# Plonky3/Plonky3

Measured on NVIDIA B200. Metric: coset_lde_batch output Gelem/s (KoalaBear 2^20 x 100 per GPU, blowup 2), higher is better.
Workload: dtype u32 (31-bit Montgomery)

## Files before the change

plonky3_b200/csrc/ntt.cu:

```cuda
#include <algorithm>
#include <cstdio>
#include <cstdlib>
#include <cstring>
#include <vector>

#include <cuda.h>

#include "common.h"

namespace p3 {

#ifdef P3GPU_NTT_PROFILE
#define P3_SKIP(flag) (flag)
#else
#define P3_SKIP(flag) false
#endif

static int env_int(const char *name, int dflt) {
    const char *s = getenv(name);
    return s ? atoi(s) : dflt;
}

struct PassArgs {
    const u32 *in;
// ... 214 lines not shown
            cp_async8(tws + k, tw + ((size_t)1 << (a.l0 + lam)) + ((size_t)T << lam) + ql);
        }
    };
    auto issue = [&](u32 t, u32 buf) {
        u32 coset, col, cw, T, ibase;
        decode(t, coset, col, cw, T, ibase);
        u32 *data = data0 + buf * buf_words;
        const u32 *in = a.in + (size_t)coset * a.in_stride + col;
        if (!shared_tw || a.n_cosets > 1) issue_twiddles(coset, T, tws0 + buf * R);
        const u32 cpr = vec16 ? (cw >> 2) : cw;
        const u32 rs = (THREADS / cpr) & ~(E2 - 1u);
        const u32 nthr = rs * cpr;
        if (rs == 0) {
            for (u32 it = threadIdx.x; it < R * cpr; it += THREADS) {
                const u32 rho = it / cpr, ch = it - rho * cpr;
                const u32 e = vec16 ? 4u * ch : ch;
                const u32 i = ibase | (rho << lowbits);
                const u32 row = a.in_bitrev ? (__brev(i) >> brsh) : i;
                u32 *dst = data + (rho >> Q2) * gstride + (rho & (E2 - 1u)) * CT + e;
                const u32 *src = in + (size_t)row * a.w + e;
                if (vec16) cp_async16(dst, src); else cp_async4(dst, src);
            }
        } else if (threadIdx.x < nthr) {
            const u32 rho0 = threadIdx.x / cpr, ch = threadIdx.x - rho0 * cpr;
            const u32 e = vec16 ? 4u * ch : ch;
            u32 *dst = data + (rho0 >> Q2) * gstride + (rho0 & (E2 - 1u)) * CT + e;
            const u32 dstep = (rs >> Q2) * gstride;
            if (!a.in_bitrev) {
                const u32 *src = in + (size_t)(ibase | (rho0 << lowbits)) * a.w + e;
                const size_t sstep = ((size_t)rs << lowbits) * a.w;
                for (u32 rho = rho0; rho < R; rho += rs, dst += dstep, src += sstep) {
                    if (vec16) cp_async16(dst, src); else cp_async4(dst, src);
                }
            } else {
                for (u32 rho = rho0; rho < R; rho += rs, dst += dstep) {
                    const u32 row = __brev(ibase | (rho << lowbits)) >> brsh;
                    const u32 *src = in + (size_t)row * a.w + e;
                    if (vec16) cp_async16(dst, src); else cp_async4(dst, src);
                }
            }
        }
        cp_async_commit();
    };

    u32 t = blockIdx.x;
    if (t >= total) return;
#ifdef P3GPU_NTT_PROFILE
#define P3_STAMP(slot) do { if (a.prof && threadIdx.x == 0 && k < 16) { unsigned long long ts_; asm volatile("mov.u64 %0, %%globaltimer;" : "=l"(ts_)); \
        a.prof[((size_t)blockIdx.x * 16 + k) * 8 + (slot)] = ts_; } } while (0)
#else
#define P3_STAMP(slot) do { } while (0)
#endif
    if (shared_tw && a.n_cosets == 1) issue_twiddles(0, 0, tws0);
    if (NBUF == 2) issue(t, 0);
    for (u32 k = 0; t < total; t += gridDim.x, k++) {
        const u32 buf = NBUF == 2 ? (k & 1u) : 0u;
        __syncthreads();
#ifdef P3GPU_NTT_PROFILE
        if (a.prof && threadIdx.x == 0 && k < 16) { u32 sm_; asm volatile("mov.u32 %0, %%smid;" : "=r"(sm_)); a.prof[((size_t)blockIdx.x * 16 + k) * 8] = sm_; }
#endif
        P3_STAMP(1);
        if (NBUF == 2) {
            if (t + gridDim.x < total) { issue(t + gridDim.x, buf ^ 1u); cp_async_wait<1>(); }
            else cp_async_wait<0>();
        } else {
            if (!P3_SKIP(a.skip_load)) issue(t, 0);
            P3_STAMP(2);
            cp_async_wait<0>();
        }
        __syncthreads();
        P3_STAMP(3);
        u32 *data = data0 + buf * buf_words;
        const uint2 *tws = (shared_tw && a.n_cosets == 1) ? tws0 : tws0 + buf * R;
        u32 coset, col, cw, T, ibase;
        decode(t, coset, col, cw, T, ibase);
        const u32 dg = THREADS / cw, dc = THREADS - dg * cw;
        {
            u32 g = threadIdx.x / cw, c = threadIdx.x - g * cw;
            for (; g < E2; ) {
                u32 *sp = data + g * CT + c;
                u32 x[E1];
#pragma unroll
                for (u32 m = 0; m < E1; m++) x[m] = sp[m * gstride];
                if (a.has_scale) {
#pragma unroll
                    for (u32 m = 0; m < E1; m++) x[m] = shoup_mul<F>(x[m], a.scale);
                }
                if (!P3_SKIP(a.skip_bfly)) reg_network<F, Q1>(x, tws, 1u);
#pragma unroll
                for (u32 m = 0; m < E1; m++) sp[m * gstride] = x[m];
                c += dc; g += dg;
                if (c >= cw) { c -= cw; g++; }
            }
        }
        __syncthreads();
        P3_STAMP(4);
        {
            u32 *out = a.out + (size_t)coset * a.out_stride + col;
            const size_t sstride = ((size_t)(a.out_bitrev ? (1u << (a.l0 + Q1)) : (1u << lowbits)) << a.out_sh) * a.w;
            u32 g = threadIdx.x / cw, c = threadIdx.x - g * cw;
            for (; g < E1; ) {
                u32 *sp = data + g * gstride + c;
                u32 x[E2];
#pragma unroll
                for (u32 m = 0; m < E2; m++) x[m] = sp[m * CT];
                if (!P3_SKIP(a.skip_bfly)) reg_network<F, Q2>(x, tws, E1 + g);
                if (a.final_reduce) {
#pragma unroll
                    for (u32 m = 0; m < E2; m++) x[m] = fp_reduce<F>(x[m]);
                }
                {
                    const u32 i0 = ibase | (g << (lowbits + Q2));
                    const u32 row0 = ((a.out_bitrev ? (__brev(i0) >> brsh) : i0) << a.out_sh) + a.out_add;
                    u32 *p = out + (size_t)row0 * a.w + c;
                    if (P3_SKIP(a.skip_store)) { u32 acc = 0;
#pragma unroll
                        for (u32 m = 0; m < E2; m++) acc ^= x[m];
                        if (acc == 0x12345678u) p[0] = acc;
                    } else if (a.out_bitrev) {
#pragma unroll
                        for (u32 m = 0; m < E2; m++) p[brev_const<Q2>(m) * sstride] = x[m];
                    } else {
#pragma unroll
                        for (u32 m = 0; m < E2; m++) p[m * sstride] = x[m];
                    }
                }
                c += dc; g += dg;
                if (c >= cw) { c -= cw; g++; }
            }
        }
        P3_STAMP(5);
    }
}

__device__ __forceinline__ void mbar_init(u32 bar, u32 count) { asm volatile("mbarrier.init.shared::cta.b64 [%0], %1;" ::"r"(bar), "r"(count)); }
__device__ __forceinline__ void mbar_wait(u32 bar, u32 parity) {
    u32 done = 0, spins = 0;
    unsigned long long t0 = 0;
    while (true) {
        asm volatile("{ .reg .pred p; mbarrier.try_wait.parity.shared::cta.b64 p, [%1], %2; selp.u32 %0, 1, 0, p; }" : "=r"(done) : "r"(bar), "r"(parity) : "memory");
        if (done) break;
        if ((++spins & 0xfffu) == 0) {
            unsigned long long now;
            asm volatile("mov.u64 %0, %%globaltimer;" : "=l"(now));
            if (t0 == 0) t0 = now;
            else if (now - t0 > 20000000000ull) __trap();
        }
    }
}
__device__ __forceinline__ void mbar_arrive(u32 bar) { asm volatile("mbarrier.arrive.shared::cta.b64 _, [%0];" ::"r"(bar) : "memory"); }
__device__ __forceinline__ void mbar_arrive_n(u32 bar, u32 n) { asm volatile("mbarrier.arrive.shared::cta.b64 _, [%0], %1;" ::"r"(bar), "r"(n) : "memory"); }
__device__ __forceinline__ void mbar_expect_tx(u32 bar, u32 bytes) { asm volatile("mbarrier.arrive.expect_tx.shared::cta.b64 _, [%0], %1;" ::"r"(bar), "r"(bytes) : "memory"); }

template <int F, int R_LOG, bool PERM, int NSTAGE, int NGROUP, int GTHREADS>
__global__ void __launch_bounds__(NGROUP * GTHREADS + 32, 1) ntt_pass_pipe_kernel(const __grid_constant__ CUtensorMap tmap, const __grid_constant__ PassArgs a) {
    constexpr u32 CT = 8;
    constexpr int Q2 = (R_LOG + 1) / 2, Q1 = R_LOG - Q2;
    constexpr u32 E1 = 1u << Q1, E2 = 1u << Q2, R = 1u << R_LOG;
    constexpr u32 GS = PERM ? E1 : E2, NG = PERM ? E2 : E1;
    constexpr u32 gstride = (GS + 1) * CT;
    constexpr u32 STAGE_WORDS = NG * gstride;
    constexpr u32 BOX_BYTES = STAGE_WORDS * 4;
    static_assert(BOX_BYTES % 128 == 0, "stage alignment");
    extern __shared__ __align__(128) unsigned char smem_raw[];
    u32 *stages = reinterpret_cast<u32 *>(smem_raw);
    uint2 *tws0 = reinterpret_cast<uint2 *>(smem_raw + (size_t)NSTAGE * BOX_BYTES);
    const u32 bar0 = (u32)__cvta_generic_to_shared(smem_raw + (size_t)NSTAGE * BOX_BYTES + 2 * R * sizeof(uint2));
    auto full_bar = [&](u32 s) { return bar0 + 8u * s; };
    auto empty_bar = [&](u32 s) { return bar0 + 8u * (NSTAGE + s); };
    auto twfull_bar = [&](u32 b) { return bar0 + 8u * (2 * NSTAGE + b); };
    auto twempty_bar = [&](u32 b) { return bar0 + 8u * (2 * NSTAGE + 2 + b); };

    if (threadIdx.x == 0) {
        for (u32 s = 0; s < NSTAGE; s++) { mbar_init(full_bar(s), 1); mbar_init(empty_bar(s), NGROUP * GTHREADS); }
        for (u32 b = 0; b < 2; b++) { mbar_init(twfull_bar(b), 1); mbar_init(twempty_bar(b), a.tpi * NGROUP * GTHREADS); }
        asm volatile("fence.mbarrier_init.release.cluster;" ::: "memory");
    }
    __syncthreads();

    const int lowbits = a.log_n - a.l1;
    const int brsh = 32 - a.log_n;
    auto decode = [&](u32 it, u32 &coset, u32 &L, u32 &T, u32 &ct0, u32 &ct1) {
        const u32 unit = it / a.csplit, chunk = it - unit * a.csplit;
        coset = unit % a.n_cosets;
        const u32 tile = unit / a.n_cosets;
        L = tile & ((1u << lowbits) - 1u);
        T = tile >> lowbits;
        ct0 = chunk * a.tpi;
        ct1 = min(ct0 + a.tpi, a.n_ctiles);
    };

    if (threadIdx.x >= NGROUP * GTHREADS) {
        if ((threadIdx.x & 31u) != 0) return;
        u32 q = 0, ui = 0;
        for (u32 it = blockIdx.x; it < a.n_items; it += gridDim.x, ui++) {
            u32 coset, L, T, ct0, ct1;
            decode(it, coset, L, T, ct0, ct1);
            const u32 b = ui & 1u, ph = (ui >> 1) & 1u;
            mbar_wait(twempty_bar(b), ph ^ 1u);
            if (ct1 - ct0 < a.tpi) mbar_arrive_n(twempty_bar(b), (a.tpi - (ct1 - ct0)) * NGROUP * GTHREADS);
            {
                const uint2 *tw = a.tw + (size_t)coset * a.tw_stride;
                uint2 *tws = tws0 + b * R;
                tws[1] = tw[((size_t)1 << a.l0) + T];
                mbar_expect_tx(twfull_bar(b), 8u * (R - 2u));
#pragma unroll 1
                for (int lam = 1; lam < R_LOG; lam++) {
                    const uint2 *src = tw + ((size_t)1 << (a.l0 + lam)) + ((size_t)T << lam);
                    asm volatile("cp.async.bulk.shared::cluster.global.mbarrier::complete_tx::bytes [%0], [%1], %2, [%3];"
                                 ::"r"((u32)__cvta_generic_to_shared(tws + (1u << lam))), "l"(src), "r"(8u << lam), "r"(twfull_bar(b)) : "memory");
                }
            }
            const u32 in_block = (a.in_tiled ? a.in_blocks > 1 : a.in_stride != 0) ? coset : 0u;
            const int blk_sh = PERM ? lowbits : a.l0;
            const int c3 = PERM ? 0 : (int)L;
            const int c4 = (PERM ? (lowbits ? (int)(__brev(L) >> (32 - lowbits)) : 0) : (int)T) + (int)(in_block << blk_sh);
            for (u32 ct = ct0; ct < ct1; ct++, q++) {
                const u32 s = q % NSTAGE, k = q / NSTAGE;
                mbar_wait(empty_bar(s), (k & 1u) ^ 1u);
                mbar_expect_tx(full_bar(s), BOX_BYTES);
                const int cc0 = a.in_tiled ? 0 : (int)(ct * CT);
                const int cc4 = a.in_tiled ? c4 + (int)((ct * a.in_blocks) << blk_sh) : c4;
                asm volatile("cp.async.bulk.tensor.5d.shared::cluster.global.mbarrier::complete_tx::bytes [%0], [%1, {%2, %3, %4, %5, %6}], [%7];"
                             ::"r"((u32)__cvta_generic_to_shared(stages + (size_t)s * STAGE_WORDS)), "l"(reinterpret_cast<unsigned long long>(&tmap)),
                               "r"(cc0), "r"(0), "r"(0), "r"(c3), "r"(cc4), "r"(full_bar(s)) : "memory");
            }
        }
        return;
    }

    const u32 gid = threadIdx.x / GTHREADS, tg = threadIdx.x - gid * GTHREADS;
    u32 q = 0, ui = 0;
#ifdef P3GPU_NTT_PROFILE
    u32 kk = 0;
#define P3_GSTAMP(slot) do { if (a.prof && tg == 0 && kk < 16) { unsigned long long ts_; asm volatile("mov.u64 %0, %%globaltimer;" : "=l"(ts_)); \
        a.prof[(((size_t)blockIdx.x * NGROUP + gid) * 16 + kk) * 8 + (slot)] = ts_; } } while (0)
#else
#define P3_GSTAMP(slot) do { } while (0)
#endif
    for (u32 it = blockIdx.x; it < a.n_items; it += gridDim.x, ui++) {
        u32 coset, L, T, ct0, ct1;
        decode(it, coset, L, T, ct0, ct1);
        const u32 b = ui & 1u, ph = (ui >> 1) & 1u;
        const uint2 *tws = tws0 + b * R;
        const u32 ibase = (a.l0 == 0 ? 0u : (T << (a.log_n - a.l0))) | L;
        bool tw_ready = false;
        for (u32 ct = ct0; ct < ct1; ct++, q++) {
            const u32 s = q % NSTAGE, k = q / NSTAGE;
            const u32 col = ct * CT, cw = min(CT, a.wc - col);
            u32 *data = stages + (size_t)s * STAGE_WORDS;
            P3_GSTAMP(1);
            mbar_wait(full_bar(s), k & 1u);
            if (!tw_ready) { mbar_wait(twfull_bar(b), ph); tw_ready = true; }
            if (q % NGROUP != gid) {
                mbar_arrive(empty_bar(s));
                mbar_arrive(twempty_bar(b));
                continue;
            }
            P3_GSTAMP(2);
            const u32 dg = GTHREADS / cw, dc = GTHREADS - dg * cw;
            {
                u32 g = tg / cw, c = tg - g * cw;
                for (; g < E2; ) {
                    u32 x[E1];
                    if (!PERM) {
                        u32 *sp = data + g * CT + c;
#pragma unroll
                        for (u32 m = 0; m < E1; m++) x[m] = sp[m * gstride];
                        if (a.has_scale) {
#pragma unroll
                            for (u32 m = 0; m < E1; m++) x[m] = shoup_mul<F>(x[m], a.scale);
                        }
                        reg_network<F, Q1>(x, tws, 1u);
#pragma unroll
                        for (u32 m = 0; m < E1; m++) sp[m * gstride] = x[m];
                    } else {
                        u32 *sp = data + g * gstride + c;
#pragma unroll
                        for (u32 m = 0; m < E1; m++) x[m] = sp[brev_const<Q1>(m) * CT];
                        if (a.has_scale) {
#pragma unroll
                            for (u32 m = 0; m < E1; m++) x[m] = shoup_mul<F>(x[m], a.scale);
                        }
                        reg_network<F, Q1>(x, tws, 1u);
#pragma unroll
                        for (u32 m = 0; m < E1; m++) sp[brev_const<Q1>(m) * CT] = x[m];
                    }
                    c += dc; g += dg;
                    if (c >= cw) { c -= cw; g++; }
                }
            }
            asm volatile("bar.sync %0, %1;" ::"r"(gid + 1u), "r"((u32)GTHREADS) : "memory");
            P3_GSTAMP(3);
            {
                const u32 ow = a.out_tiled ? CT : a.w;
                u32 *out = a.out_tiled ? a.out + ((((size_t)ct * a.n_cosets + coset) << a.log_n) << 3) : a.out + (size_t)coset * a.out_stride + col;
                const size_t sstride = ((size_t)(a.out_bitrev ? (1u << (a.l0 + Q1)) : (1u << lowbits)) << a.out_sh) * ow;
                u32 g = tg / cw, c = tg - g * cw;
                bool released = false;
                for (; g < E1; ) {
                    u32 x[E2];
                    u32 gg;
                    if (!PERM) {
                        gg = g;
                        const u32 *sp = data + g * gstride + c;
#pragma unroll
                        for (u32 m = 0; m < E2; m++) x[m] = sp[m * CT];
                    } else {
                        gg = __brev(g) >> (32 - Q1);
                        const u32 *sp = data + g * CT + c;
#pragma unroll
                        for (u32 m = 0; m < E2; m++) x[m] = sp[brev_const<Q2>(m) * gstride];
                    }
                    u32 gn = g + dg, cn = c + dc;
                    if (cn >= cw) { cn -= cw; gn++; }
                    if (gn >= E1) {
                        asm volatile("fence.proxy.async.shared::cta;" ::: "memory");
                        mbar_arrive(empty_bar(s));
                        released = true;
                    }
                    reg_network<F, Q2>(x, tws, E1 + gg);
                    if (a.final_reduce) {
#pragma unroll
                        for (u32 m = 0; m < E2; m++) x[m] = fp_reduce<F>(x[m]);
                    }
                    const u32 i0 = ibase | (gg << (lowbits + Q2));
                    const u32 row0 = ((a.out_bitrev ? (__brev(i0) >> brsh) : i0) << a.out_sh) + a.out_add;
                    u32 *p = out + (size_t)row0 * ow + c;
                    if (a.shard_log_rows) {
                        const u32 grow = (coset << a.log_n) + row0;
                        p = a.shard_out[grow >> a.shard_log_rows] + (size_t)(grow & ((1u << a.shard_log_rows) - 1u)) * ow + col + c;
                    }
                    if (a.out_bitrev) {
#pragma unroll
                        for (u32 m = 0; m < E2; m++) p[brev_const<Q2>(m) * sstride] = x[m];
                    } else {
#pragma unroll
                        for (u32 m = 0; m < E2; m++) p[m * sstride] = x[m];
                    }
                    g = gn; c = cn;
                }
                if (!released) {
                    asm volatile("fence.proxy.async.shared::cta;" ::: "memory");
                    mbar_arrive(empty_bar(s));
                }
            }
            mbar_arrive(twempty_bar(b));
            P3_GSTAMP(4);
#ifdef P3GPU_NTT_PROFILE
            kk++;
#endif
        }
    }
}

struct TwGenArgs {
    u32 sigma[32];
    u32 roots[32];
};
template <int F> __global__ void gen_twiddle_heap(uint2 *Z, int log_n, const TwGenArgs a) {
    const size_t idx = (size_t)blockIdx.x * blockDim.x + threadIdx.x;
    if (idx >= ((size_t)1 << log_n)) return;
    if (idx == 0) { Z[0] = make_uint2(0, 0); return; }
    const int l = 63 - __clzll((long long)idx);
    const u32 q = (u32)(idx - ((size_t)1 << l));
    u32 z = a.sigma[l];
    for (int b = 0; b < l; b++)
        if ((q >> b) & 1u) z = mont_mul<F>(z, a.roots[b + 2]);
    Z[idx] = shoup_pair<F>(from_monty<F>(z));
}

struct PowArgs { u32 pw[32]; };
template <int F> __global__ void scale_rows_by_powers(u32 *m, size_t h, size_t w, const PowArgs a) {
    const size_t idx = (size_t)blockIdx.x * blockDim.x + threadIdx.x;
    if (idx >= h * w) return;
    size_t row = idx / w;
    u32 s = Fp<F>::ONE;
    for (int k = 0; row; k++, row >>= 1)
        if (row & 1) s = mont_mul<F>(s, a.pw[k]);
    m[idx] = mont_mul<F>(m[idx], s);
}
__global__ void broadcast_row(const u32 *in, u32 *out, size_t rows, size_t w) {
    const size_t idx = (size_t)blockIdx.x * blockDim.x + threadIdx.x;
    if (idx < rows * w) out[idx] = in[idx % w];
}

template <int F>
static int32_t get_twiddles(p3gpu_ctx *ctx, int log_n, int added_bits, u32 shift, int inverse, const uint2 **out) {
    TwiddleKey key{F, log_n, shift, inverse + 2 * added_bits};
    std::lock_guard<std::recursive_mutex> g(ctx->call_mu);
    {
        auto it = ctx->twiddles.find(key);
        if (it != ctx->twiddles.end()) { it->second.last_use = ctx->tick; *out = it->second.ptr; return P3GPU_OK; }
    }
    const size_t N = (size_t)1 << log_n, n_cosets = (size_t)1 << added_bits;
    const size_t bytes = n_cosets * N * sizeof(uint2);
    while (ctx->twiddle_bytes + bytes > ctx->twiddle_cap_bytes) {
        auto victim = ctx->twiddles.end();
        for (auto it = ctx->twiddles.begin(); it != ctx->twiddles.end(); ++it)
            if (it->second.last_use < ctx->tick && (victim == ctx->twiddles.end() || it->second.last_use < victim->second.last_use)) victim = it;
        if (victim == ctx->twiddles.end()) break;
        P3_CUDA(cudaStreamSynchronize(ctx->stream));
        P3_CUDA(cudaFree(victim->second.ptr));
        ctx->twiddle_bytes -= victim->second.bytes;
        ctx->twiddles.erase(victim);
    }
    uint2 *Z = nullptr;
    {
        cudaError_t e = cudaMalloc(&Z, bytes);
        if (e != cudaSuccess) { set_error("cudaMalloc(%zu) for a twiddle heap failed: %s", bytes, cudaGetErrorString(e)); cudaGetLastError(); return P3GPU_ENOMEM; }
    }
    const u32 g_big = two_adic_generator<F>((u32)(log_n + added_bits));
    for (size_t cb = 0; cb < n_cosets; cb++) {
        size_t c = 0;
        for (int b = 0; b < added_bits; b++) c |= ((cb >> b) & 1) << (added_bits - 1 - b);
        const u32 s = mont_mul<F>(shift, fp_pow<F>(g_big, c));
        TwGenArgs a;
        for (int l = 0; l < 32; l++) { a.sigma[l] = Fp<F>::ONE; a.roots[l] = Fp<F>::ONE; }
        for (int l = 0; l < log_n; l++) a.sigma[l] = fp_pow<F>(s, (u64)(N >> (l + 1)));
        for (u32 k = 0; k <= (u32)log_n && k <= Fp<F>::TWO_ADICITY; k++) {
            u32 gk = two_adic_generator<F>(k);
            a.roots[k] = inverse ? fp_inv<F>(gk) : gk;
        }
        const unsigned blocks = (unsigned)((N + 255) / 256);
        gen_twiddle_heap<F><<<blocks, 256, 0, ctx->stream>>>(Z + cb * N, log_n, a);
        ctx->launches++;
        const cudaError_t e = cudaGetLastError();
        if (e != cudaSuccess) { cudaFree(Z); set_error("gen_twiddle_heap launch failed: %s", cudaGetErrorString(e)); return P3GPU_ECUDA; }
    }
    ctx->twiddles.emplace(key, TwiddleEntry{Z, bytes, ctx->tick});
    ctx->twiddle_bytes += bytes;
    *out = Z;
    return P3GPU_OK;
}

template <int F, int LOG_CT, bool VEC>
static int32_t launch_pass_ct(p3gpu_ctx *ctx, const PassArgs &a) {
    constexpr int THREADS = 256;
    const int r = a.l1 - a.l0;
    const size_t smem = (((size_t)1 << r) << LOG_CT) * 4 + ((size_t)1 << r) * sizeof(uint2);
    auto kern = ntt_pass_kernel<F, LOG_CT, THREADS, VEC>;
    if (smem > 48 * 1024) P3_CUDA(cudaFuncSetAttribute(kern, cudaFuncAttributeMaxDynamicSharedMemorySize, (int)smem));
    const size_t tiles = ((size_t)1 << (a.log_n - r)) * a.n_ctiles * a.n_cosets;
    P3_CHECK(tiles < (1ull << 31), P3GPU_EINVAL, "ntt: grid too large");
    kern<<<(unsigned)tiles, THREADS, smem, ctx->stream>>>(a);
    ctx->launches++;
    P3_CUDA(cudaGetLastError());
    return P3GPU_OK;
}

template <int F, int R_LOG, int CT_T, int THREADS, int NBUF>
static int32_t launch_fast_rct(p3gpu_ctx *ctx, const PassArgs &a) {
    constexpr int Q2 = (R_LOG + 1) / 2, Q1 = R_LOG - Q2;
    const u32 ct = a.ct;
    const u32 e2 = 1u << Q2, e1 = 1u << Q1;
    const u32 padw = (ct + 32u - ((e2 * ct) & 31u)) & 31u;
    const size_t buf_words = ((size_t)e1 * (e2 * ct + padw) + 3) & ~(size_t)3;
    const size_t smem = NBUF * buf_words * 4 + NBUF * ((size_t)1 << R_LOG) * sizeof(uint2);
    auto kern = ntt_pass_fast_kernel<F, R_LOG, CT_T, THREADS, NBUF>;
    P3_CHECK(smem <= 227 * 1024, P3GPU_EINVAL, "ntt: tile does not fit shared memory");
    static size_t smem_set[64] = {0};
    if (smem > 48 * 1024 && smem > smem_set[ctx->device & 63]) {
        P3_CUDA(cudaFuncSetAttribute(kern, cudaFuncAttributeMaxDynamicSharedMemorySize, (int)smem));
        smem_set[ctx->device & 63] = smem;
    }
    const size_t tiles = ((size_t)1 << (a.log_n - R_LOG)) * a.n_ctiles * a.n_cosets;
    P3_CHECK(tiles < (1ull << 31), P3GPU_EINVAL, "ntt: grid too large");
    size_t per_sm = std::min<size_t>(NBUF == 1 ? 2048 / THREADS : 2, (227 * 1024) / (smem + 1024));
    static int num_regs = 0;
    if (num_regs == 0) {
        cudaFuncAttributes fa;
        P3_CUDA(cudaFuncGetAttributes(&fa, kern));
        num_regs = std::max(fa.numRegs, 16);
    }
    const size_t by_regs = 65536 / ((size_t)THREADS * (size_t)num_regs);
    if (per_sm > by_regs) per_sm = by_regs;
    if (per_sm < 1) per_sm = 1;
    const size_t grid = std::min(tiles, per_sm * (size_t)ctx->sm_count);
    kern<<<(unsigned)grid, THREADS, smem, ctx->stream>>>(a);
    ctx->launches++;
    P3_CUDA(cudaGetLastError());
    return P3GPU_OK;
}
template <int F, int R_LOG, int CT_T>
static int32_t launch_fast_rc(p3gpu_ctx *ctx, const PassArgs &a) {
    static const int threads = env_int("P3GPU_NTT_THREADS", 256);
    if (threads == 512) return launch_fast_rct<F, R_LOG, CT_T, 512, 2>(ctx, a);
    return launch_fast_rct<F, R_LOG, CT_T, 256, 1>(ctx, a);
}
template <int F, int R_LOG>
static int32_t launch_fast_r(p3gpu_ctx *ctx, const PassArgs &a) {
    switch (a.ct) {
        case 16: return launch_fast_rc<F, R_LOG, 16>(ctx, a);
        case 20: return launch_fast_rc<F, R_LOG, 20>(ctx, a);
        case 24: return launch_fast_rc<F, R_LOG, 24>(ctx, a);
        default: return launch_fast_rc<F, R_LOG, 0>(ctx, a);
    }
}
template <int F>
static int32_t launch_fast(p3gpu_ctx *ctx, const PassArgs &a) {
    switch (a.l1 - a.l0) {
        case 6: return launch_fast_r<F, 6>(ctx, a);
        case 7: return launch_fast_r<F, 7>(ctx, a);
        case 8: return launch_fast_r<F, 8>(ctx, a);
        case 9: return launch_fast_r<F, 9>(ctx, a);
        default: return launch_fast_r<F, 10>(ctx, a);
    }
}

typedef CUresult (*TensorMapEncodeFn)(CUtensorMap *, CUtensorMapDataType, cuuint32_t, void *, const cuuint64_t *, const cuuint64_t *,
                                      const cuuint32_t *, const cuuint32_t *, CUtensorMapInterleave, CUtensorMapSwizzle,
                                      CUtensorMapL2promotion, CUtensorMapFloatOOBfill);
static TensorMapEncodeFn tensor_map_encoder() {
    static TensorMapEncodeFn fn = []() -> TensorMapEncodeFn {
        void *p = nullptr;
        cudaDriverEntryPointQueryResult qres;
        if (cudaGetDriverEntryPoint("cuTensorMapEncodeTiled", &p, cudaEnableDefault, &qres) != cudaSuccess || qres != cudaDriverEntryPointSuccess)
            return nullptr;
        return reinterpret_cast<TensorMapEncodeFn>(p);
    }();
    return fn;
}

static int32_t make_pass_tensor_map(const PassArgs &a, bool perm, CUtensorMap *tm) {
    TensorMapEncodeFn enc = tensor_map_encoder();
    P3_CHECK(enc != nullptr, P3GPU_ECUDA, "cuTensorMapEncodeTiled is not available from this driver");
    const int r = a.l1 - a.l0, q2 = (r + 1) / 2, q1 = r - q2, lowbits = a.log_n - a.l1;
    const cuuint64_t pitch = a.in_tiled ? 32 : (cuuint64_t)a.w * 4;
    const cuuint64_t n_ctiles = (a.wc + 7) / 8;
    cuuint64_t dims[5], strides[4];
    cuuint32_t box[5] = {8, 0, 0, 1, 1}, es[5] = {1, 1, 1, 1, 1};
    dims[0] = a.in_tiled ? 8 : a.wc;
    const cuuint64_t in_blocks = a.in_tiled ? n_ctiles * a.in_blocks : (a.in_stride ? a.n_cosets : 1);
    if (!perm) {
        dims[1] = 1ull << q2; dims[2] = 1ull << q1; dims[3] = 1ull << lowbits; dims[4] = in_blocks << a.l0;
        strides[0] = pitch << lowbits; strides[1] = pitch << (lowbits + q2); strides[2] = pitch; strides[3] = pitch << (a.log_n - a.l0);
        box[1] = (1u << q2) + 1; box[2] = 1u << q1;
    } else {
        dims[1] = 1ull << q1; dims[2] = 1ull << q2; dims[3] = 1; dims[4] = in_blocks << (a.log_n - r);
        strides[0] = pitch; strides[1] = pitch << q1; strides[2] = pitch; strides[3] = pitch << r;
        box[1] = (1u << q1) + 1; box[2] = 1u << q2;
    }
    const CUresult rc = enc(tm, CU_TENSOR_MAP_DATA_TYPE_UINT32, 5, const_cast<u32 *>(a.in), dims, strides, box, es, CU_TENSOR_MAP_INTERLEAVE_NONE,
                            CU_TENSOR_MAP_SWIZZLE_NONE, CU_TENSOR_MAP_L2_PROMOTION_L2_128B, CU_TENSOR_MAP_FLOAT_OOB_FILL_NONE);
    P3_CHECK(rc == CUDA_SUCCESS, P3GPU_ECUDA, "cuTensorMapEncodeTiled failed (%d)", (int)rc);
    return P3GPU_OK;
}

static bool pipe_eligible(const PassArgs &a) {
    if (!env_int("P3GPU_NTT_PIPE", 1)) return false;
    const int r = a.l1 - a.l0;
    if (r < 6 || r > 10) return false;
    if (a.in_tiled || a.out_tiled) return true;
    if (a.w % 4 != 0 || a.w < 8 || a.w > 8192) return false;
    if (reinterpret_cast<uintptr_t>(a.in) % 16 != 0) return false;
    if ((((size_t)a.w * 4) << a.log_n) >= (1ull << 40)) return false;
    if (a.in_stride != 0 && a.in_stride != ((size_t)a.w << a.log_n)) return false;
    if (a.in_bitrev && (a.l0 != 0 || (a.in_stride != 0 && a.n_cosets > 1))) return false;
    return true;
}

template <int F, int R_LOG, bool PERM>
static int32_t launch_pipe_r(p3gpu_ctx *ctx, PassArgs a) {
    constexpr int NSTAGE = 6, NGROUP = 4, GTHREADS = 128;
    constexpr int Q2 = (R_LOG + 1) / 2, Q1 = R_LOG - Q2;
    constexpr size_t GS = PERM ? (1u << Q1) : (1u << Q2), NG = PERM ? (1u << Q2) : (1u << Q1);
    constexpr size_t box_bytes = NG * (GS + 1) * 8 * 4;
    constexpr size_t smem = NSTAGE * box_bytes + 2 * ((size_t)1 << R_LOG) * sizeof(uint2) + (2 * NSTAGE + 4) * 8;
    static_assert(smem <= 227 * 1024, "pipelined NTT kernel: shared memory budget");
    CUtensorMap tm;
    if (a.wc == 0) a.wc = a.w;
    if (a.in_blocks == 0) a.in_blocks = 1;
    P3_TRY(make_pass_tensor_map(a, PERM, &tm));
    a.n_ctiles = (a.wc + 7) / 8;
    const size_t units = ((size_t)1 << (a.log_n - R_LOG)) * a.n_cosets;
    size_t csplit = units >= 2 * (size_t)ctx->sm_count ? 1 : std::min<size_t>(a.n_ctiles, (2 * (size_t)ctx->sm_count + units - 1) / units);
    a.tpi = (u32)((a.n_ctiles + csplit - 1) / csplit);
    csplit = (a.n_ctiles + a.tpi - 1) / a.tpi;
    a.csplit = (u32)csplit;
    const size_t items = units * csplit;
    P3_CHECK(items < (1ull << 31), P3GPU_EINVAL, "ntt: too many tiles");
    P3_CHECK((size_t)a.tpi * NGROUP * GTHREADS < (1u << 20), P3GPU_EINVAL, "ntt: too many column tiles per unit for the mbarrier count");
    a.n_items = (u32)items;
    auto kern = ntt_pass_pipe_kernel<F, R_LOG, PERM, NSTAGE, NGROUP, GTHREADS>;
    static bool attr_set[64] = {false};
    if (!attr_set[ctx->device & 63]) {
        P3_CUDA(cudaFuncSetAttribute(kern, cudaFuncAttributeMaxDynamicSharedMemorySize, (int)smem));
        attr_set[ctx->device & 63] = true;
    }
    const size_t grid = std::min(items, (size_t)ctx->sm_count);
    kern<<<(unsigned)grid, NGROUP * GTHREADS + 32, smem, ctx->stream>>>(tm, a);
    ctx->launches++;
    P3_CUDA(cudaGetLastError());
    return P3GPU_OK;
}
template <int F, int R_LOG>
static int32_t launch_pipe_p(p3gpu_ctx *ctx, const PassArgs &a) {
    return a.in_bitrev ? launch_pipe_r<F, R_LOG, true>(ctx, a) : launch_pipe_r<F, R_LOG, false>(ctx, a);
}
template <int F>
static int32_t launch_pipe(p3gpu_ctx *ctx, const PassArgs &a) {
    switch (a.l1 - a.l0) {
        case 6: return launch_pipe_p<F, 6>(ctx, a);
        case 7: return launch_pipe_p<F, 7>(ctx, a);
        case 8: return launch_pipe_p<F, 8>(ctx, a);
        case 9: return launch_pipe_p<F, 9>(ctx, a);
        default: return launch_pipe_p<F, 10>(ctx, a);
    }
}

static u32 choose_tile_width(u32 w) {
    if (w <= 24) return w;
    static const int forced = env_int("P3GPU_NTT_CT", 0);
    if (forced) return (u32)forced;
    for (u32 ct : {16u, 20u, 24u, 12u})
        if (w % ct == 0) return ct;
    const u32 n = (w + 19) / 20;
    u32 ct = (w + n - 1) / n;
    ct = (ct + 3) & ~3u;
    return ct > 24 ? 24 : ct;
}

template <int F>
static int32_t launch_pass(p3gpu_ctx *ctx, PassArgs a, unsigned n_cosets, int main_log_ct) {
    a.n_cosets = n_cosets;
    const int r = a.l1 - a.l0;
#ifdef P3GPU_NTT_PROFILE
    {
        static int launch_no = 0;
        const char *pb = getenv("P3GPU_NTT_PROFBUF");
        a.prof = pb ? reinterpret_cast<unsigned long long *>(strtoull(pb, nullptr, 0)) + (size_t)(launch_no++ % 8) * (1u << 17) : nullptr;
    }
#endif
    if (!env_int("P3GPU_NTT_GENERIC", 0) && pipe_eligible(a)) return launch_pipe<F>(ctx, a);
    if (r >= 6 && r <= 10 && !env_int("P3GPU_NTT_GENERIC", 0)) {
        const u32 ct = choose_tile_width(a.w);
        const bool al16 = (a.w % 4 == 0) && (ct % 4 == 0) &&
                          ((reinterpret_cast<uintptr_t>(a.in) | reinterpret_cast<uintptr_t>(a.out)) % 16 == 0) &&
                          ((a.in_stride | a.out_stride) % 4 == 0);
        a.col0 = 0; a.ct = ct; a.n_ctiles = (a.w + ct - 1) / ct; a.vec16 = al16;
        a.skip_bfly = env_int("P3GPU_NTT_NOBFLY", 0);
        a.skip_load = env_int("P3GPU_NTT_NOLOAD", 0); a.skip_store = env_int("P3GPU_NTT_NOSTORE", 0);
        return launch_fast<F>(ctx, a);
    }
    const bool aligned = (a.w % 4 == 0) && ((reinterpret_cast<uintptr_t>(a.in) | reinterpret_cast<uintptr_t>(a.out)) % 16 == 0) &&
                         ((a.in_stride | a.out_stride) % 4 == 0);
    u32 col = 0, rem = a.w;
    for (int lct = main_log_ct; lct >= 0 && rem; lct--) {
        const u32 ct = 1u << lct;
        const u32 n = rem >> lct;
        if (!n) continue;
        a.col0 = col; a.n_ctiles = n; a.ct = ct;
        const bool vec = aligned && lct >= 2 && (col % 4 == 0);
        int32_t rc;
        switch (lct) {
            case 5: rc = vec ? launch_pass_ct<F, 5, true>(ctx, a) : launch_pass_ct<F, 5, false>(ctx, a); break;
            case 4: rc = vec ? launch_pass_ct<F, 4, true>(ctx, a) : launch_pass_ct<F, 4, false>(ctx, a); break;
            case 3: rc = vec ? launch_pass_ct<F, 3, true>(ctx, a) : launch_pass_ct<F, 3, false>(ctx, a); break;
            case 2: rc = vec ? launch_pass_ct<F, 2, true>(ctx, a) : launch_pass_ct<F, 2, false>(ctx, a); break;
            case 1: rc = launch_pass_ct<F, 1, false>(ctx, a); break;
            default: rc = launch_pass_ct<F, 0, false>(ctx, a); break;
        }
        P3_TRY(rc);
        col += n * ct; rem -= n * ct;
    }
    return P3GPU_OK;
}

struct ShardedOut {
    unsigned world, log_rows;
    u32 *out[16];
    size_t w_total, col_off;
};

struct NetworkPlan {
    int n_passes;
    int bounds[8];
};
static NetworkPlan plan_passes(int log_n, int max_r) {
    NetworkPlan p;
    p.n_passes = (log_n + max_r - 1) / max_r;
    if (p.n_passes < 1) p.n_passes = 1;
    int base = log_n / p.n_passes, extra = log_n % p.n_passes;
    p.bounds[0] = 0;
    for (int k = 0; k < p.n_passes; k++) p.bounds[k + 1] = p.bounds[k] + base + (k < extra ? 1 : 0);
    return p;
}

template <int F>
static int32_t run_network(p3gpu_ctx *ctx, int log_n, size_t w, const uint2 *tw, size_t tw_stride, unsigned n_cosets,
                           const u32 *src, size_t src_stride, int in_bitrev, u32 *dst, size_t dst_stride, int out_bitrev,
                           int out_sh, u32 out_add, u32 *tmp, bool has_scale, uint2 scale, bool final_reduce) {
    const int max_r = std::min(12, std::max(4, env_int("P3GPU_NTT_MAXR", 10)));
    const int main_log_ct = std::min(5, std::max(0, env_int("P3GPU_NTT_LOGCT", 4)));
    const NetworkPlan plan = plan_passes(log_n, max_r);
    const bool remap = out_bitrev || out_sh != 0 || out_add != 0;
    const size_t hw = ((size_t)1 << log_n) * w;
    if (remap && plan.n_passes > 1) P3_CHECK(tmp != nullptr, P3GPU_EINVAL, "ntt: scratch missing");
    for (int k = 0; k < plan.n_passes; k++) {
        PassArgs a;
        memset(&a, 0, sizeof a);
        const bool first = (k == 0), last = (k == plan.n_passes - 1);
        a.w = (u32)w; a.log_n = log_n; a.l0 = plan.bounds[k]; a.l1 = plan.bounds[k + 1];
        a.tw = tw; a.tw_stride = tw_stride;
        u32 *mid = remap ? tmp : dst;
        const size_t mid_stride = remap ? hw : dst_stride;
        a.in = first ? src : mid;
        a.in_stride = first ? src_stride : mid_stride;
        a.in_bitrev = first ? in_bitrev : 0;
        if (last) {
            a.out = dst; a.out_stride = dst_stride;
            a.out_bitrev = out_bitrev; a.out_sh = out_sh; a.out_add = out_add;
            a.final_reduce = final_reduce;
        } else {
            a.out = mid; a.out_stride = mid_stride;
        }
        if (first) { a.has_scale = has_scale; a.scale = scale; }
        P3_TRY(launch_pass<F>(ctx, a, n_cosets, main_log_ct));
    }
    return P3GPU_OK;
}

template <int F> static uint2 inv_height_scale(size_t h) {
    return shoup_pair<F>(from_monty<F>(fp_inv<F>(to_monty<F>((u32)(h % Fp<F>::P)))));
}

template <int F>
static int32_t dft_batch_impl(p3gpu_ctx *ctx, int kind, const u32 *d_in, u32 *d_out, size_t h, size_t w, u32 shift) {
    const int log_n = (int)log2_floor(h);
    if (log_n == 0) {
        if (d_in != d_out) P3_CUDA(cudaMemcpyAsync(d_out, d_in, w * 4, cudaMemcpyDeviceToDevice, ctx->stream));
        return P3GPU_OK;
    }
    const bool inverse = (kind == P3GPU_IDFT || kind == P3GPU_COSET_IDFT);
    const u32 tw_shift = (kind == P3GPU_COSET_DFT) ? shift : Fp<F>::ONE;
    const uint2 *tw = nullptr;
    P3_TRY(get_twiddles<F>(ctx, log_n, 0, tw_shift, inverse, &tw));
    void *tmp = nullptr;
    P3_TRY(ctx_scratch(ctx, h * w * 4, &tmp));
    P3_TRY(run_network<F>(ctx, log_n, w, tw, 0, 1, d_in, 0, 0, d_out, 0, 1, 0, 0, (u32 *)tmp, inverse,
                          inverse ? inv_height_scale<F>(h) : make_uint2(0, 0), true));
    if (kind == P3GPU_COSET_IDFT) {
        PowArgs pa;
        u32 b = fp_inv<F>(shift);
        for (int k = 0; k < 32; k++) { pa.pw[k] = b; b = mont_mul<F>(b, b); }
        const size_t n = h * w;
        scale_rows_by_powers<F><<<(unsigned)((n + 255) / 256), 256, 0, ctx->stream>>>(d_out, h, w, pa);
// ... 244 lines not shown
```

Before: 132.5.

## Store NTT pass output via TMA bulk tensor copy from shared memory

```diff
diff --git a/plonky3_b200/csrc/ntt.cu b/plonky3_b200/csrc/ntt.cu
--- a/plonky3_b200/csrc/ntt.cu
+++ b/plonky3_b200/csrc/ntt.cu
@@ -390,8 +390,9 @@
 __device__ __forceinline__ void mbar_arrive_n(u32 bar, u32 n) { asm volatile("mbarrier.arrive.shared::cta.b64 _, [%0], %1;" ::"r"(bar), "r"(n) : "memory"); }
 __device__ __forceinline__ void mbar_expect_tx(u32 bar, u32 bytes) { asm volatile("mbarrier.arrive.expect_tx.shared::cta.b64 _, [%0], %1;" ::"r"(bar), "r"(bytes) : "memory"); }
 
-template <int F, int R_LOG, bool PERM, int NSTAGE, int NGROUP, int GTHREADS>
-__global__ void __launch_bounds__(NGROUP * GTHREADS + 32, 1) ntt_pass_pipe_kernel(const __grid_constant__ CUtensorMap tmap, const __grid_constant__ PassArgs a) {
+template <int F, int R_LOG, bool PERM, int NSTAGE, int NGROUP, int GTHREADS, bool TST>
+__global__ void __launch_bounds__(NGROUP * GTHREADS + 32, 1) ntt_pass_pipe_kernel(const __grid_constant__ CUtensorMap tmap, const __grid_constant__ CUtensorMap omap,
+                                                                                  const __grid_constant__ PassArgs a) {
     constexpr u32 CT = 8;
     constexpr int Q2 = (R_LOG + 1) / 2, Q1 = R_LOG - Q2;
     constexpr u32 E1 = 1u << Q1, E2 = 1u << Q2, R = 1u << R_LOG;
@@ -400,6 +401,7 @@
     constexpr u32 STAGE_WORDS = NG * gstride;
     constexpr u32 BOX_BYTES = STAGE_WORDS * 4;
     static_assert(BOX_BYTES % 128 == 0, "stage alignment");
+    static_assert(!(PERM && TST), "a PERM stage is not in the output box layout");
     extern __shared__ __align__(128) unsigned char smem_raw[];
     u32 *stages = reinterpret_cast<u32 *>(smem_raw);
     uint2 *tws0 = reinterpret_cast<uint2 *>(smem_raw + (size_t)NSTAGE * BOX_BYTES);
@@ -530,7 +532,35 @@
             }
             asm volatile("bar.sync %0, %1;" ::"r"(gid + 1u), "r"((u32)GTHREADS) : "memory");
             P3_GSTAMP(3);
-            {
+            if (TST) {
+                u32 g = tg / cw, c = tg - g * cw;
+                for (; g < E1; ) {
+                    u32 *sp = data + g * gstride + c;
+                    u32 x[E2];
+#pragma unroll
+                    for (u32 m = 0; m < E2; m++) x[m] = sp[m * CT];
+                    reg_network<F, Q2>(x, tws, E1 + g);
+                    if (a.final_reduce) {
+#pragma unroll
+                        for (u32 m = 0; m < E2; m++) x[m] = fp_reduce<F>(x[m]);
+                    }
+#pragma unroll
+                    for (u32 m = 0; m < E2; m++) sp[m * CT] = x[m];
+                    c += dc; g += dg;
+                    if (c >= cw) { c -= cw; g++; }
+                }
+                asm volatile("fence.proxy.async.shared::cta;" ::: "memory");
+                asm volatile("bar.sync %0, %1;" ::"r"(gid + 1u), "r"((u32)GTHREADS) : "memory");
+                if (tg == 0) {
+                    const u32 blk = a.out_tiled ? ct * a.n_cosets + coset : coset;
+                    asm volatile("cp.async.bulk.tensor.5d.global.shared::cta.bulk_group [%0, {%1, %2, %3, %4, %5}], [%6];"
+                                 ::"l"(reinterpret_cast<unsigned long long>(&omap)), "r"(a.out_tiled ? 0 : (int)col), "r"(0), "r"(0), "r"((int)L),
+                                   "r"((int)(T + (blk << a.l0))), "r"((u32)__cvta_generic_to_shared(data)) : "memory");
+                    asm volatile("cp.async.bulk.commit_group;" ::: "memory");
+                    asm volatile("cp.async.bulk.wait_group.read 0;" ::: "memory");
+                }
+                mbar_arrive(empty_bar(s));
+            } else {
                 const u32 ow = a.out_tiled ? CT : a.w;
                 u32 *out = a.out_tiled ? a.out + ((((size_t)ct * a.n_cosets + coset) << a.log_n) << 3) : a.out + (size_t)coset * a.out_stride + col;
                 const size_t sstride = ((size_t)(a.out_bitrev ? (1u << (a.l0 + Q1)) : (1u << lowbits)) << a.out_sh) * ow;
@@ -590,6 +620,7 @@
 #endif
         }
     }
+    if (TST && tg == 0) asm volatile("cp.async.bulk.wait_group 0;" ::: "memory");
 }
 
 struct TwGenArgs {
@@ -785,6 +816,31 @@
     return P3GPU_OK;
 }
 
+static bool pass_out_tma_ok(const PassArgs &a) {
+    if (!env_int("P3GPU_NTT_TMA_STORE", 1)) return false;
+    if (a.in_bitrev || a.out_bitrev || a.out_sh || a.out_add || a.shard_log_rows) return false;
+    if (a.out_tiled) return true;
+    const size_t pitch = (size_t)a.w * 4;
+    if (pitch % 16 != 0 || reinterpret_cast<uintptr_t>(a.out) % 16 != 0) return false;
+    if (a.n_cosets > 1 && a.out_stride != ((size_t)a.w << a.log_n)) return false;
+    return ((pitch << a.log_n) * a.n_cosets) < (1ull << 40);
+}
+
+static int32_t make_pass_out_tensor_map(const PassArgs &a, CUtensorMap *tm) {
+    TensorMapEncodeFn enc = tensor_map_encoder();
+    P3_CHECK(enc != nullptr, P3GPU_ECUDA, "cuTensorMapEncodeTiled is not available from this driver");
+    const int r = a.l1 - a.l0, q2 = (r + 1) / 2, q1 = r - q2, lowbits = a.log_n - a.l1;
+    const cuuint64_t pitch = a.out_tiled ? 32 : (cuuint64_t)a.w * 4;
+    const cuuint64_t blocks = a.out_tiled ? (cuuint64_t)((a.wc + 7) / 8) * a.n_cosets : a.n_cosets;
+    cuuint64_t dims[5] = {a.out_tiled ? 8 : (cuuint64_t)a.wc, 1ull << q2, 1ull << q1, 1ull << lowbits, blocks << a.l0};
+    cuuint64_t strides[4] = {pitch << lowbits, pitch << (lowbits + q2), pitch, pitch << (a.log_n - a.l0)};
+    cuuint32_t box[5] = {8, (1u << q2) + 1, 1u << q1, 1, 1}, es[5] = {1, 1, 1, 1, 1};
+    const CUresult rc = enc(tm, CU_TENSOR_MAP_DATA_TYPE_UINT32, 5, a.out, dims, strides, box, es, CU_TENSOR_MAP_INTERLEAVE_NONE,
+                            CU_TENSOR_MAP_SWIZZLE_NONE, CU_TENSOR_MAP_L2_PROMOTION_L2_128B, CU_TENSOR_MAP_FLOAT_OOB_FILL_NONE);
+    P3_CHECK(rc == CUDA_SUCCESS, P3GPU_ECUDA, "cuTensorMapEncodeTiled (output) failed (%d)", (int)rc);
+    return P3GPU_OK;
+}
+
 static bool pipe_eligible(const PassArgs &a) {
     if (!env_int("P3GPU_NTT_PIPE", 1)) return false;
     const int r = a.l1 - a.l0;
@@ -798,18 +854,18 @@
     return true;
 }
 
-template <int F, int R_LOG, bool PERM>
-static int32_t launch_pipe_r(p3gpu_ctx *ctx, PassArgs a) {
+template <int F, int R_LOG, bool PERM, bool TST>
+static int32_t launch_pipe_rt(p3gpu_ctx *ctx, PassArgs a) {
     constexpr int NSTAGE = 6, NGROUP = 4, GTHREADS = 128;
     constexpr int Q2 = (R_LOG + 1) / 2, Q1 = R_LOG - Q2;
     constexpr size_t GS = PERM ? (1u << Q1) : (1u << Q2), NG = PERM ? (1u << Q2) : (1u << Q1);
     constexpr size_t box_bytes = NG * (GS + 1) * 8 * 4;
     constexpr size_t smem = NSTAGE * box_bytes + 2 * ((size_t)1 << R_LOG) * sizeof(uint2) + (2 * NSTAGE + 4) * 8;
     static_assert(smem <= 227 * 1024, "pipelined NTT kernel: shared memory budget");
-    CUtensorMap tm;
-    if (a.wc == 0) a.wc = a.w;
-    if (a.in_blocks == 0) a.in_blocks = 1;
+    CUtensorMap tm, om;
+    memset(&om, 0, sizeof om);
     P3_TRY(make_pass_tensor_map(a, PERM, &tm));
+    if (TST) P3_TRY(make_pass_out_tensor_map(a, &om));
     a.n_ctiles = (a.wc + 7) / 8;
     const size_t units = ((size_t)1 << (a.log_n - R_LOG)) * a.n_cosets;
     size_t csplit = units >= 2 * (size_t)ctx->sm_count ? 1 : std::min<size_t>(a.n_ctiles, (2 * (size_t)ctx->sm_count + units - 1) / units);
@@ -820,17 +876,24 @@
     P3_CHECK(items < (1ull << 31), P3GPU_EINVAL, "ntt: too many tiles");
     P3_CHECK((size_t)a.tpi * NGROUP * GTHREADS < (1u << 20), P3GPU_EINVAL, "ntt: too many column tiles per unit for the mbarrier count");
     a.n_items = (u32)items;
-    auto kern = ntt_pass_pipe_kernel<F, R_LOG, PERM, NSTAGE, NGROUP, GTHREADS>;
+    auto kern = ntt_pass_pipe_kernel<F, R_LOG, PERM, NSTAGE, NGROUP, GTHREADS, TST>;
     static bool attr_set[64] = {false};
     if (!attr_set[ctx->device & 63]) {
         P3_CUDA(cudaFuncSetAttribute(kern, cudaFuncAttributeMaxDynamicSharedMemorySize, (int)smem));
         attr_set[ctx->device & 63] = true;
     }
     const size_t grid = std::min(items, (size_t)ctx->sm_count);
-    kern<<<(unsigned)grid, NGROUP * GTHREADS + 32, smem, ctx->stream>>>(tm, a);
+    kern<<<(unsigned)grid, NGROUP * GTHREADS + 32, smem, ctx->stream>>>(tm, om, a);
     ctx->launches++;
     P3_CUDA(cudaGetLastError());
     return P3GPU_OK;
+}
+template <int F, int R_LOG, bool PERM>
+static int32_t launch_pipe_r(p3gpu_ctx *ctx, PassArgs a) {
+    if (a.wc == 0) a.wc = a.w;
+    if (a.in_blocks == 0) a.in_blocks = 1;
+    if (!PERM && pass_out_tma_ok(a)) return launch_pipe_rt<F, R_LOG, false, true>(ctx, a);
+    return launch_pipe_rt<F, R_LOG, PERM, false>(ctx, a);
 }
 template <int F, int R_LOG>
 static int32_t launch_pipe_p(p3gpu_ctx *ctx, const PassArgs &a) {
```

New measurement: 137.5, median of 6. 1.04x the previous value.
